# saurabh260918/Graph-Attention-Network-GATv2-

Hardware: AMD Instinct MI355X
Metric: edges/sec (fwd+bwd, 2-layer 8-head GATv2) (higher is better)
Workload: dtype f32; 1 GPU; products-shape synthetic power-law graph, 2450000 nodes / 61900000 edges / 100 feat / 47 classes, 2-layer GATv2 heads [8, 8] outdims [8, 8], fp32; launch=eager, parallelism=single GPU, generator=device (csrc/gat_synth.hip), bit-for-bit synth.py

## Files before the change

### graph-attention-network-gatv2-_amd/csrc/gat_abi.hip

```cpp
#include "gat_internal.h"

#include <algorithm>
#include <cmath>
#include <cstdlib>
#include <cstring>
#include <memory>
#include <mutex>

namespace gat {

static thread_local std::string g_err;
void set_error(const std::string& msg) { g_err = msg; }
int fail(int code, const std::string& msg) {
    g_err = msg;
    return code ? code : GAT_E_INVALID;
}
static std::mutex g_choice_mu;
static std::vector<std::pair<std::string, std::string>> g_choices;
const char* choice_env(const char* name) {
    const char* e = getenv(name);
    if (e) {
        std::lock_guard<std::mutex> lock(g_choice_mu);
        bool seen = false;
        for (auto& kv : g_choices) if (kv.first == name) { kv.second = e; seen = true; }
// ... 935 lines not shown
static bool fused_head(gat_ctx* c) {
    if (c->cfg.keep_taps) return false;
    HeadArgs f{}; HeadBwdArgs b{};
    head_args(c, &f, &b);
    return head_step_supported(b);
}
static int head_step(gat_ctx* c, bool with_gh = true) {
    HeadArgs f{}; HeadBwdArgs b{};
    head_args(c, &f, &b);
    if (!with_gh) b.gh_out = nullptr;
    Scope t(c, GAT_K_HEAD_BWD);
    c->y_valid = false;
    return launch_head_step(f, b, c->stream);
}
static bool fused_last(gat_ctx* c) {
    if (!fused_head(c) || bf16(c) || c->comm || c->n_table != c->n_rows || c->cfg.flat_lrelu_index) return false;
    const Layer& y = c->layers.back();
    if (!edge_fast_path(y.H, y.D, c->n_table) || !y.stash || c->stash == nullptr || c->gH == nullptr) return false;
    if (!edge_last_fused_supported(y.H, y.D, c->cfg.num_classes) || c->dbg != 0) return false;
    static const int env = [] { const char* e = choice_env("GAT_FUSE_LAST"); return e ? (e[0] == '0' ? 0 : 1) : 0; }();
    return env == 1;
}
static int last_layer_fused(gat_ctx* c) {
    const int l = c->cfg.num_layers - 1;
    Layer& y = c->layers[l];
    BwdPlan P;
    GAT_TRY(plan_backward_edges(c, l, &P));
    const EdgeFwdArgs f = plan_forward_edges(c, l);
    const int32_t n_seg = c->work.n_slots;
    float* ga_a = P.a.ga_partial;
    int blocks_a = 0;
    if (n_seg > 0) {
        EdgeFwdArgs fs = f;
        fs.n_items = n_seg;
        {
            Scope t(c, GAT_K_EDGE_FWD);
            GAT_TRY(launch_edge_forward(fs, c->stream));
        }
        {
            Scope t(c, GAT_K_HEAD_BWD);
            GAT_TRY(launch_head_rows(c->slot_info, c->work.n_slots, c->work.n_split, Wo_of(c), y.hout, c->labels_eff ? c->labels_eff : c->labels,
                                     c->gH, c->gh_stride, c->cfg.num_classes, y.D, c->stream));
        }
        EdgeBwdArgs bs = P.a;
        bs.n_items = n_seg;
        bs.ga_partial = ga_a;
        bs.ga_blocks = blocks_a = std::min(1024, edge_backward_blocks(n_seg, y.H, y.D, P.store, false, false, P.stash));
        Scope t(c, GAT_K_EDGE_BWD);
        GAT_TRY(launch_edge_backward(bs, c->stream));
    }
    EdgeLastArgs a{};
    a.f = f; a.f.items = c->items + n_seg; a.f.n_items = c->work.n_items - n_seg;
    float* ga_b = ga_a + (int64_t)blocks_a * y.HD;
    a.b = P.a; a.b.ga_partial = ga_b; a.b.ga_blocks = a.f.n_items > 0 ? std::min(edge_last_fused_blocks(a.f.n_items), 2048 - blocks_a) : 0;
    a.Wo = Wo_of(c); a.labels = c->labels_eff ? c->labels_eff : c->labels; a.gh_out = c->gH; a.C = c->cfg.num_classes;
    {
        Scope t(c, GAT_K_EDGE_FUSED);
        GAT_TRY(launch_edge_last_fused(a, c->stream));
    }
    GAT_TRY(head_step(c, false));
    GAT_TRY(sum_backward_edges(c, l, P));
    Scope t(c, GAT_K_MISC);
    return launch_reduce_partials_add(ga_a, blocks_a + a.b.ga_blocks, y.HD, ga_of(c, l), c->stream);
}
static int overlap_prepare(gat_ctx* c) {
    static const int env = [] { const char* e = choice_env("GAT_OVERLAP"); return e ? (e[0] == '0' ? 0 : 1) : -1; }();
    const int L = c->cfg.num_layers;
    const bool want = env == 1;
    if (!want || L < 2 || c->gPL_bound || c->Xtab) return 0;
    if (!c->gPL_alt) {
        hipStreamCaptureStatus cs = hipStreamCaptureStatusNone;
        (void)hipStreamIsCapturing(c->stream, &cs);
        if (cs != hipStreamCaptureStatusNone) return 0;
        GAT_TRY(dalloc(c, &c->gPL_alt, c->n_table * c->HDmax));
        GAT_TRY(dalloc(c, &c->gPR_alt, c->n_rows * c->HDmax));
        {
            int least = 0, greatest = 0;
            (void)hipDeviceGetStreamPriorityRange(&least, &greatest);
            static const bool prio = [] { const char* e = choice_env("GAT_OVERLAP_PRIO"); return !(e && e[0] == '0'); }();
            if (prio) GAT_HIP(hipStreamCreateWithPriority(&c->side_stream, hipStreamNonBlocking, least));
            else GAT_HIP(hipStreamCreateWithFlags(&c->side_stream, hipStreamNonBlocking));
        }
        for (int l = 0; l < L; ++l) {
            hipEvent_t a, b;
            GAT_HIP(hipEventCreateWithFlags(&a, hipEventDisableTiming));
            GAT_HIP(hipEventCreateWithFlags(&b, hipEventDisableTiming));
            c->ev_fork.push_back(a); c->ev_join.push_back(b);
        }
    }
    return 1;
}
struct OverlapScope {
    gat_ctx* c;
    explicit OverlapScope(gat_ctx* c_, bool on) : c(c_) { c->ov_active = on; }
    ~OverlapScope() { c->ov_active = false; }
};
static int backward_phases(gat_ctx* c, bool head_done = false, bool last_edges_done = false) {
    const int L = c->cfg.num_layers;
    const int ov = last_edges_done ? 0 : overlap_prepare(c);
    if (ov < 0) return ov;
    OverlapScope scope(c, ov == 1);
    std::vector<char> forked((size_t)L, 0);
    if (!head_done) GAT_TRY(gat_head_backward(c));
    for (int l = L - 1; l >= 0; --l) {
        if (ov && l + 2 < L && forked[(size_t)l + 2]) {
            GAT_HIP(hipStreamWaitEvent(c->stream, c->ev_join[(size_t)l + 2], 0));
            forked[(size_t)l + 2] = 0;
// ... 573 lines not shown
```

### graph-attention-network-gatv2-_amd/csrc/gat_edge_kernels.hip

```cpp
#include "gat_internal.h"

#include <map>
#include <mutex>

namespace gat {
namespace {

constexpr float kLog2e = 1.4426950408889634f;
constexpr float kLn2 = 0.6931471805599453f;

__device__ __forceinline__ float lrelu(float v, float s) { return v > 0.f ? v : v * s; }
__device__ __forceinline__ float exp2_fast(float x) { return __builtin_amdgcn_exp2f(x); }

template <int CTRL>
__device__ __forceinline__ float dpp_mov(float v) {
    return __builtin_bit_cast(
        float, __builtin_amdgcn_update_dpp(0, __builtin_bit_cast(int, v), CTRL, 0xF, 0xF, true));
}

template <int D>
__device__ __forceinline__ float group_sum(float t) {
    if constexpr (D >= 2) t += dpp_mov<0xB1>(t);
    if constexpr (D >= 4) t += dpp_mov<0x4E>(t);
    if constexpr (D >= 8) t += dpp_mov<0x141>(t);
// ... 942 lines not shown
            for (int u = 0; u < U; ++u) al[u] = hsum<N>(ac2 * lrelu_n<N>(v[u] + pr, A.slope));
            group_sum_n<DL, U>(al);
#pragma unroll
            for (int u = 0; u < U; ++u) {
                al[u] = exp2_fast(al[u] - m2) * inv;
                ga_[u] = hsum<N>(g * v[u]);
            }
            group_sum_n<DL, U>(ga_);
#pragma unroll
            for (int u = 0; u < U; ++u) {
                const bool valid = b + st * U + u < e;
                const float ge = valid ? al[u] * (ga_[u] - dot) : 0.f;
                const vnf<N> s = v[u] + pr;
                const vnf<N> gs = ge * select_pos<N>(s, ac, acs);
                ga += ge * lrelu_n<N>(s, A.slope);
                gpr += gs;
                if constexpr (MSG) {
                    pend_m[u] = g * al[u] + gs;
                } else {
                    uint32_t bits = 0;
#pragma unroll
                    for (int i = 0; i < N; ++i) bits |= (s[i] > 0.f ? 1u : 0u) << i;
                    const uint32_t w = __builtin_bit_cast(uint32_t, (cp & 1) ? ge : al[u]);
                    pend_w[u] = ((w + (1u << (N - 1))) & ~((1u << N) - 1u)) | bits;
                }
            }
        }
        if constexpr (MSG) {
            if constexpr (DBG != 1) {
#pragma unroll
                for (int u = 0; u < U; ++u) store_row_n<HD, N, BF>(A.msg, (int)pend_s[u], cp, pend_m[u]);
            }
        } else if constexpr (DBG != 1 && DBG != 3) {
#pragma unroll
            for (int u = 0; u < U; ++u) stream_store(&A.stash[(uint64_t)pend_s[u] * LPE + cp], pend_w[u]);
        }
        if (row >= 0) {
            float* dst = slot < 0 ? A.gPR + rowc * HD + c : A.part_acc + (int64_t)slot * HD + c;
            stream_store(reinterpret_cast<vnf<N>*>(dst), gpr);
        }
    }
#pragma unroll
    for (int off = LPE; off < 64; off <<= 1) ga += shfl_xor_n<N>(ga, off);
    if (gidx == 0) {
#pragma unroll
        for (int i = 0; i < N; ++i) red[wave][c + i] = ga[i];
    }
    __syncthreads();
    if (threadIdx.x < HD)
        A.ga_partial[(int64_t)blockIdx.x * HD + threadIdx.x] =
            (red[0][threadIdx.x] + red[1][threadIdx.x]) + (red[2][threadIdx.x] + red[3][threadIdx.x]);
}

template <int HD, int D, int N>
__global__ __launch_bounds__(256) __attribute__((amdgpu_waves_per_eu(4, 8))) void edge_last_fused_kernel(EdgeLastArgs A) {
    constexpr int LPE = HD / N, G = 64 / LPE, DL = D / N, H = HD / D;
    constexpr int U = 4, JC = 4;
    static_assert(LPE == 16 && DL == 2 && D == 8 && N == 4, "16 lanes per row, two lanes per head, D = 8");
    __shared__ float red[4][HD];
    __shared__ float s_wo[64 * D];
    const EdgeFwdArgs& F = A.f;
    const EdgeBwdArgs& B = A.b;
    const int C = A.C;
    for (int i = threadIdx.x; i < C * D; i += blockDim.x) s_wo[i] = A.Wo[i];
    __syncthreads();
    const int lane = threadIdx.x & 63;
    const int wave = __builtin_amdgcn_readfirstlane(threadIdx.x >> 6);
    const int cp = lane % LPE, gidx = lane / LPE;
    const int c = N * cp;
    const vnf<N> ac = *reinterpret_cast<const vnf<N>*>(F.a + c);
    const vnf<N> acs = ac * F.slope;
    const vnf<N> ac2 = ac * kLog2e;
    const int64_t nquads = (F.n_items + G - 1) / G;
    const int64_t nwaves = (int64_t)gridDim.x * 4;
    vnf<N> ga = vzero<N>();

    for (int64_t q = (int64_t)blockIdx.x * 4 + wave; q < nquads; q += nwaves) {
        const int64_t it = q * G + gidx;
        int row = -1, b = 0, e = 0;
        if (it < F.n_items) { const int4 item = F.items[it]; row = item.x; b = item.y; e = item.z; }
        const int64_t rowc = row < 0 ? 0 : row;
        const int nst = wave_max_over_groups<HD, N>((e - b + U - 1) / U);
        const vnf<N> pr = *reinterpret_cast<const vnf<N>*>(F.PR + rowc * HD + c);
        float m = -1e9f * kLog2e, Z = 0.f;
        vnf<N> acc = vzero<N>();
        {
            auto load_src = [&](int st) {
                int j = b + st * U + (cp & (U - 1));
                j = j < e ? j : e - 1;
                return F.col_idx[j > 0 ? j : 0];
            };
            int srcv = load_src(0);
            for (int st = 0; st < nst; ++st) {
                const int srcn = load_src(st + 1);
                vnf<N> v[U];
#pragma unroll
                for (int u = 0; u < U; ++u) v[u] = gather_row_n<HD, N, false>(F.PL, __shfl(srcv, gidx * LPE + u), cp);
                float t[U];
#pragma unroll
                for (int u = 0; u < U; ++u) t[u] = hsum<N>(ac2 * lrelu_n<N>(v[u] + pr, F.slope));
                group_sum_n<DL, U>(t);
                float cm = -INFINITY;
#pragma unroll
                for (int u = 0; u < U; ++u) {
                    t[u] = (b + st * U + u < e) ? t[u] : -INFINITY;
                    cm = fmaxf(cm, t[u]);
                }
                const float mn = fmaxf(m, cm);
                const float scale = exp2_fast(m - mn);
                Z *= scale;
                acc = acc * scale;
#pragma unroll
                for (int u = 0; u < U; ++u) {
                    const float p = exp2_fast(t[u] - mn);
                    Z += p;
                    acc += p * v[u];
                }
                m = mn;
                srcv = srcn;
            }
        }
        const float inv = __builtin_amdgcn_rcpf(Z + 1e-8f);
        const vnf<N> hp = acc * inv;
        if (row >= 0) {
            stream_store(reinterpret_cast<vnf<N>*>(F.hpre + rowc * HD + c), hp);
            if ((c % D) == 0) { F.mstat[rowc * H + c / D] = m; F.zstat[rowc * H + c / D] = Z; }
        }
        vnf<N> hm = lrelu_n<N>(hp, F.slope);
#pragma unroll
        for (int off = DL; off < LPE; off <<= 1) hm += shfl_xor_n<N>(hm, off);
        hm = hm / (float)H;
        if (row >= 0 && cp < DL) *reinterpret_cast<vnf<N>*>(F.hout + rowc * D + c) = hm;
        const vnf<N> ho_other = shfl_xor_n<N>(hm, 1);
        float ho[D];
#pragma unroll
        for (int k = 0; k < N; ++k) { ho[k] = (cp & 1) ? ho_other[k] : hm[k]; ho[N + k] = (cp & 1) ? hm[k] : ho_other[k]; }
        const int lab = A.labels[rowc];
        float z[JC], mv = -INFINITY;
#pragma unroll
        for (int j = 0; j < JC; ++j) {
            const int cls = cp + LPE * j;
            z[j] = -INFINITY;
            if (cls < C) {
                float t = 0.f;
#pragma unroll
                for (int d = 0; d < D; ++d) t += s_wo[cls * D + d] * ho[d];
                z[j] = t;
                mv = fmaxf(mv, t);
            }
        }
#pragma unroll
        for (int off = 1; off < LPE; off <<= 1) mv = fmaxf(mv, __shfl_xor(mv, off));
        float ev[JC], sum = 0.f;
#pragma unroll
        for (int j = 0; j < JC; ++j) { ev[j] = (cp + LPE * j < C) ? exp2_fast((z[j] - mv) * kLog2e) : 0.f; sum += ev[j]; }
        sum = group_sum<LPE>(sum);
        const float rden = 1.0f / (sum + 1e-8f);
        float gh[D];
#pragma unroll
        for (int d = 0; d < D; ++d) gh[d] = 0.f;
#pragma unroll
        for (int j = 0; j < JC; ++j) {
            const int cls = cp + LPE * j;
            if (cls < C) {
                const float dz = lab >= 0 ? ev[j] * rden - (cls == lab ? 1.0f : 0.0f) : 0.0f;
#pragma unroll
                for (int d = 0; d < D; ++d) gh[d] += s_wo[cls * D + d] * dz;
            }
        }
        group_sum_n<LPE, D>(gh);
        vnf<N> ghl;
#pragma unroll
        for (int k = 0; k < N; ++k) ghl[k] = (cp & 1) ? gh[N + k] : gh[k];
        if (row >= 0 && cp < DL) *reinterpret_cast<vnf<N>*>(A.gh_out + rowc * B.gh_stride + c) = ghl;
        vnf<N> dsel;
#pragma unroll
        for (int i = 0; i < N; ++i) dsel[i] = hp[i] > 0.f ? 1.0f : F.slope;
        const vnf<N> g = ghl * dsel * (1.0f / (float)H);
        if (row >= 0) {
            if (B.hbits != nullptr) {
                uint32_t nib = 0;
#pragma unroll
                for (int i = 0; i < N; ++i) nib |= (hp[i] > 0.f ? 1u : 0u) << i;
                B.hbits[rowc * B.hb_stride + cp] = (uint8_t)nib;
            } else {
                stream_store(reinterpret_cast<vnf<N>*>(B.gfull + rowc * HD + c), g);
            }
        }
        const float dot = group_sum<DL>(hsum<N>(g * hp));
        const float m2 = m;
        auto load_idx = [&](int st, int& srcv, int& posv) {
            int j = b + st * U + (cp & (U - 1));
            j = j < e ? j : e - 1;
            j = j > 0 ? j : 0;
            srcv = B.col_idx[j];
            posv = B.pos[j];
        };
        auto spread = [&](int st, int srcv, int posv, int (&src)[U], uint32_t (&sl)[U]) {
#pragma unroll
            for (int u = 0; u < U; ++u) {
                src[u] = __shfl(srcv, gidx * LPE + u);
                const uint32_t p = (uint32_t)__shfl(posv, gidx * LPE + u);
                sl[u] = (b + st * U + u < e) ? p : B.stash_spare;
            }
        };
        int srcv, posv, srcn, posn;
        load_idx(0, srcv, posv);
        load_idx(1, srcn, posn);
        vnf<N> gpr = vzero<N>();
        int src[U];
        uint32_t sl[U], pend_s[U], pend_w[U];
        spread(0, srcv, posv, src, sl);
#pragma unroll
        for (int u = 0; u < U; ++u) { pend_w[u] = 0u; pend_s[u] = B.stash_spare; }
        for (int st = 0; st < nst; ++st) {
            vnf<N> v[U];
#pragma unroll
            for (int u = 0; u < U; ++u) v[u] = gather_row_n<HD, N, false>(B.PL, src[u], cp);
#pragma unroll
            for (int u = 0; u < U; ++u) stream_store(&B.stash[(uint64_t)pend_s[u] * LPE + cp], pend_w[u]);
#pragma unroll
            for (int u = 0; u < U; ++u) pend_s[u] = sl[u];
            spread(st + 1, srcn, posn, src, sl);
            load_idx(st + 2, srcn, posn);
            float al[U], ga_[U];
#pragma unroll
            for (int u = 0; u < U; ++u) al[u] = hsum<N>(ac2 * lrelu_n<N>(v[u] + pr, F.slope));
            group_sum_n<DL, U>(al);
#pragma unroll
            for (int u = 0; u < U; ++u) {
                al[u] = exp2_fast(al[u] - m2) * inv;
                ga_[u] = hsum<N>(g * v[u]);
            }
            group_sum_n<DL, U>(ga_);
#pragma unroll
            for (int u = 0; u < U; ++u) {
                const bool valid = b + st * U + u < e;
                const float ge = valid ? al[u] * (ga_[u] - dot) : 0.f;
                const vnf<N> s = v[u] + pr;
                const vnf<N> gs = ge * select_pos<N>(s, ac, acs);
                ga += ge * lrelu_n<N>(s, F.slope);
                gpr += gs;
                uint32_t bits = 0;
#pragma unroll
                for (int i = 0; i < N; ++i) bits |= (s[i] > 0.f ? 1u : 0u) << i;
                const uint32_t w = __builtin_bit_cast(uint32_t, (cp & 1) ? ge : al[u]);
                pend_w[u] = ((w + (1u << (N - 1))) & ~((1u << N) - 1u)) | bits;
            }
        }
#pragma unroll
        for (int u = 0; u < U; ++u) stream_store(&B.stash[(uint64_t)pend_s[u] * LPE + cp], pend_w[u]);
        if (row >= 0) stream_store(reinterpret_cast<vnf<N>*>(B.gPR + rowc * HD + c), gpr);
    }
#pragma unroll
    for (int off = LPE; off < 64; off <<= 1) ga += shfl_xor_n<N>(ga, off);
    if (gidx == 0) {
#pragma unroll
        for (int i = 0; i < N; ++i) red[wave][c + i] = ga[i];
    }
    __syncthreads();
    if (threadIdx.x < HD)
        B.ga_partial[(int64_t)blockIdx.x * HD + threadIdx.x] =
            (red[0][threadIdx.x] + red[1][threadIdx.x]) + (red[2][threadIdx.x] + red[3][threadIdx.x]);
}

__global__ __launch_bounds__(256) void head_rows_kernel(const int4* __restrict__ slot_info, int32_t n_slots, int32_t n_split,
                                                       const float* __restrict__ Wo, const float* __restrict__ HL,
                                                       const int32_t* __restrict__ labels, float* __restrict__ gh_out,
                                                       int32_t gh_stride, int32_t C, int32_t DLAST) {
    const int k = blockIdx.x * blockDim.x + threadIdx.x;
    if (k >= n_split) return;
    const int64_t row = slot_info[slot_info[n_slots + k].x].x;
    const float* x = HL + row * DLAST;
    const int lab = labels[row];
    float mv = -INFINITY;
    for (int c = 0; c < C; ++c) {
        float t = 0.f;
        for (int d = 0; d < DLAST; ++d) t += Wo[c * DLAST + d] * x[d];
        mv = fmaxf(mv, t);
    }
    float sum = 0.f;
    for (int c = 0; c < C; ++c) {
        float t = 0.f;
        for (int d = 0; d < DLAST; ++d) t += Wo[c * DLAST + d] * x[d];
        sum += exp2_fast((t - mv) * kLog2e);
    }
    const double rden = 1.0 / ((double)sum + 1e-8);
    float acc[16];
    for (int d = 0; d < DLAST; ++d) acc[d] = 0.f;
    for (int c = 0; c < C; ++c) {
        float t = 0.f;
        for (int d = 0; d < DLAST; ++d) t += Wo[c * DLAST + d] * x[d];
        const float y = (float)((double)exp2_fast((t - mv) * kLog2e) * rden);
        const float dz = lab >= 0 ? y - (c == lab ? 1.0f : 0.0f) : 0.0f;
        for (int d = 0; d < DLAST; ++d) acc[d] += Wo[c * DLAST + d] * dz;
    }
    for (int d = 0; d < DLAST; ++d) gh_out[row * gh_stride + d] = acc[d];
}

#ifdef GAT_EXPERIMENTS
template <int NCW, int R>
struct RecRing {
    uint32_t rec[NCW][R][16 * 16];
    uint32_t slot[NCW][R][16];
    int head[NCW], tail[NCW], done[NCW];
// ... 576 lines not shown
    const int dummy = 0;
    auto probe = [&]() -> int {
        GAT_DISPATCH_HD_D(stash_words_t, dummy, nullptr)
        return 0;
    };
    return probe();
}

int edge_backward_blocks(int64_t n_items, int32_t H, int32_t D_, bool store, bool taps, bool bf16, bool stash) {
    int64_t want = (n_items + 3) / 4;
    if (want < 1) want = 1;
    const int HD = H * D_, D = D_;
    const BwdSel sel{store, taps, bf16, stash};
    auto cap = [&]() -> int {
        GAT_DISPATCH_HD_D(bwd_resident, sel, nullptr)
        return 2048;
    };
    int c = cap();
#ifdef GAT_EXPERIMENTS
    static const int dbg = [] { const char* e = getenv("GAT_DBG"); return e ? atoi(e) : 0; }();
    if (dbg == 4 && HD == 64 && D == 8 && stash && !bf16 && !taps) c = c / 2;
#endif
    return (int)(want < c ? want : c);
}

static int fast_probe(const int&, hipStream_t) { return 1; }
template <int HD, int D>
int fast_probe_t(const int& x, hipStream_t s) { return fast_probe(x, s); }

bool edge_fast_path(int32_t H, int32_t D_, int64_t n_table) {
    const int HD = H * D_, D = D_;
    if (n_table * HD * (int64_t)sizeof(float) >= ((int64_t)1 << 32)) return false;
    const int dummy = 0;
    auto probe = [&]() -> int {
        GAT_DISPATCH_HD_D(fast_probe_t, dummy, nullptr)
        return 0;
    };
    return probe() == 1;
}

int launch_edge_backward(const EdgeBwdArgs& a, hipStream_t s) {
    const int HD = a.H * a.D, D = a.D;
    if (a.ga_blocks < 1) return fail(GAT_E_INVALID, "edge_backward: ga_blocks must come from edge_backward_blocks()");
    if (edge_fast_path(a.H, a.D, a.n_table)) { GAT_DISPATCH_HD_D(run_bwd, a, s) }
    if (a.pos != nullptr) return fail(GAT_E_INVALID, "edge_backward: the generic path has no store mode");
    const size_t lds = (size_t)(3 * a.H + 2 * HD) * sizeof(float);
    if (lds > 64 * 1024) return fail(GAT_E_UNSUPPORTED, "edge_backward: H*D too large for the generic path");
    hipLaunchKernelGGL(edge_bwd_generic, dim3((unsigned)a.ga_blocks), dim3(64), lds, s, a);
    GAT_HIP(hipGetLastError());
    return 0;
}

bool edge_last_fused_supported(int32_t H, int32_t D, int32_t C) { return H * D == 64 && D == 8 && C >= 1 && C <= 64; }
int edge_last_fused_blocks(int64_t n_items) {
    const int64_t want = std::max<int64_t>(1, ((n_items + 3) / 4 + 3) / 4);
    const int cap = resident_blocks((const void*)edge_last_fused_kernel<64, 8, 4>);
    return (int)std::min<int64_t>(want, cap);
}
int launch_edge_last_fused(const EdgeLastArgs& a, hipStream_t s) {
    if (!edge_last_fused_supported(a.f.H, a.f.D, a.C)) return fail(GAT_E_UNSUPPORTED, "edge_last_fused: shape outside the kernel");
    if (a.f.n_items <= 0) return 0;
    if (a.f.items == nullptr || a.b.pos == nullptr || a.b.stash == nullptr || a.gh_out == nullptr || a.b.ga_blocks < 1 ||
        (a.b.hbits == nullptr && a.b.gfull == nullptr))
        return fail(GAT_E_INVALID, "edge_last_fused: missing buffers");
    hipLaunchKernelGGL((edge_last_fused_kernel<64, 8, 4>), dim3((unsigned)a.b.ga_blocks), dim3(256), 0, s, a);
    GAT_HIP(hipGetLastError());
    return 0;
}
int launch_head_rows(const int4* slot_info, int32_t n_slots, int32_t n_split, const float* Wo, const float* HL, const int32_t* labels,
                     float* gh_out, int32_t gh_stride, int32_t C, int32_t DLAST, hipStream_t s) {
    if (n_split <= 0) return 0;
    if (DLAST > 16) return fail(GAT_E_UNSUPPORTED, "head_rows: D_last > 16");
    hipLaunchKernelGGL(head_rows_kernel, dim3((unsigned)((n_split + 255) / 256)), dim3(256), 0, s, slot_info, n_slots, n_split, Wo, HL,
                       labels, gh_out, gh_stride, C, DLAST);
    GAT_HIP(hipGetLastError());
    return 0;
}

int launch_csr_to_coo(const int32_t* row_ptr, const int32_t* col_idx, int32_t* src, int32_t* dst,
                      int64_t n_rows, int64_t n_edges, int64_t dst_offset, hipStream_t s) {
    if (n_edges <= 0) return 0;
    int64_t blocks = (n_edges + 255) / 256;
    if (blocks > 65536) blocks = 65536;
    hipLaunchKernelGGL(csr_to_coo_kernel, dim3((unsigned)blocks), dim3(256), 0, s, row_ptr, col_idx, src,
                       dst, n_rows, n_edges, (int32_t)dst_offset);
    GAT_HIP(hipGetLastError());
    return 0;
}

static int launch_transpose(const float* src, float* dst, int64_t A_, int64_t B_, hipStream_t s) {
    const int64_t total = A_ * B_;
    if (total <= 0) return 0;
    int64_t blocks = (total + 255) / 256;
    if (blocks > 65536) blocks = 65536;
    hipLaunchKernelGGL(transpose_kernel, dim3((unsigned)blocks), dim3(256), 0, s, src, dst, A_, B_);
    GAT_HIP(hipGetLastError());
    return 0;
}
int launch_transpose_eh_to_he(const float* src_eh, float* dst_he, int64_t E, int32_t H, hipStream_t s) {
    return launch_transpose(src_eh, dst_he, E, H, s);
}
int launch_transpose_he_to_eh(const float* src_he, float* dst_eh, int64_t E, int32_t H, hipStream_t s) {
    return launch_transpose(src_he, dst_eh, H, E, s);
}
int launch_transpose_nh_to_hn(const float* src_nh, float* dst_hn, int64_t N, int32_t H, hipStream_t s) {
    return launch_transpose(src_nh, dst_hn, N, H, s);
}

}
```

### graph-attention-network-gatv2-_amd/csrc/gat_gemm_kernels.hip

```cpp
#include "gat_internal.h"

#include <cstdlib>
#include <map>
#include <mutex>
#include <utility>

namespace gat {
namespace {

typedef float v16f __attribute__((ext_vector_type(16)));

struct ASrcRows {
    const float* X; int32_t ld;
    __device__ __forceinline__ float4 load4(int64_t i, int k) const {
        return *reinterpret_cast<const float4*>(X + i * ld + k);
    }
    __device__ __forceinline__ float load1(int64_t i, int k) const { return X[i * ld + k]; }
};
struct ASrcGcat {
    const float* gPL; const float* gPR; int32_t HD;
    __device__ __forceinline__ float4 load4(int64_t i, int k) const {
        return k < HD ? *reinterpret_cast<const float4*>(gPL + i * HD + k)
                      : *reinterpret_cast<const float4*>(gPR + i * HD + (k - HD));
    }
// ... 24 lines not shown
    __device__ __forceinline__ void apply(int64_t i, int j, float v, float) const { (*this)(i, j, v); }
    __device__ __forceinline__ void operator()(int64_t i, int j, float v) const {
        j += j0;
        if (j < HD) {
            if constexpr (BF) {
                const uint32_t u = __builtin_bit_cast(uint32_t, v);
                reinterpret_cast<uint16_t*>(PL)[i * HD + j] = (uint16_t)((u + 0x7FFFu + ((u >> 16) & 1u)) >> 16);
            } else {
                PL[i * HD + j] = v;
            }
        } else {
            PR[i * HD + (j - HD)] = v;
        }
    }
};
struct EpiGradX {
    static constexpr bool kTwoPhase = true;
    float* out; const float* hpre_prev; int32_t ld; float slope;
    __device__ __forceinline__ float pre(int64_t i, int j) const { return hpre_prev[i * ld + j]; }
    __device__ __forceinline__ void apply(int64_t i, int j, float v, float hv) const {
        out[i * ld + j] = v * (hv > 0.f ? 1.0f : slope);
    }
    __device__ __forceinline__ void operator()(int64_t i, int j, float v) const { apply(i, j, v, pre(i, j)); }
};

struct EpiStore {
    static constexpr bool kTwoPhase = false;
    float* out; int32_t ld;
    __device__ __forceinline__ float pre(int64_t, int) const { return 0.f; }
    __device__ __forceinline__ void apply(int64_t i, int j, float v, float) const { out[i * ld + j] = v; }
    __device__ __forceinline__ void operator()(int64_t i, int j, float v) const { out[i * ld + j] = v; }
};

constexpr int kKC = 128;

}

int64_t resident_blocks(const void* fn, size_t dyn_lds, int threads) {
    static std::mutex mu;
    static std::map<std::pair<const void*, size_t>, int64_t> cache;
    std::lock_guard<std::mutex> lock(mu);
    const auto key = std::make_pair(fn, dyn_lds);
    auto it = cache.find(key);
    if (it != cache.end()) return it->second;
    int per_cu = 0, dev = 0, cus = 256;
    if (hipOccupancyMaxActiveBlocksPerMultiprocessor(&per_cu, fn, threads, dyn_lds) != hipSuccess || per_cu < 1) per_cu = 1;
    if (per_cu > 8) per_cu = 8;
    (void)hipGetDevice(&dev);
    (void)hipDeviceGetAttribute(&cus, hipDeviceAttributeMultiprocessorCount, dev);
    (void)hipGetLastError();
    return cache[key] = (int64_t)per_cu * (cus > 0 ? cus : 256);
}

static void allow_big_lds(const void* fn) {
    static std::mutex mu;
    static std::map<std::pair<const void*, int>, bool> done;
    int dev = 0;
    (void)hipGetDevice(&dev);
    std::lock_guard<std::mutex> lock(mu);
    bool& d = done[std::make_pair(fn, dev)];
    if (!d) { (void)hipFuncSetAttribute(fn, hipFuncAttributeMaxDynamicSharedMemorySize, 160 * 1024); (void)hipGetLastError(); d = true; }
}

namespace {

template <int NT, bool VEC4, class AS, class BS, class EP>
__global__ __launch_bounds__(256) void rowgemm_kernel(AS as, BS bs, EP ep, int64_t M, int32_t N, int32_t K,
                                                      int32_t kc_lds) {
    constexpr int NW = NT * 32;
    extern __shared__ float Bsh[];
    const int lane = threadIdx.x & 63, wave = threadIdx.x >> 6;
    const int li = lane & 31, half = lane >> 5;
    const int n0 = blockIdx.y * NW;
    const int64_t ntiles = (M + 127) / 128;
    bool b_loaded = false;
    for (int64_t tile = blockIdx.x; tile < ntiles; tile += gridDim.x) {
        const int64_t row = tile * 128 + wave * 32 + li;
        const bool rvalid = row < M;
        v16f acc[NT];
#pragma unroll
        for (int nt = 0; nt < NT; ++nt)
#pragma unroll
            for (int r = 0; r < 16; ++r) acc[nt][r] = 0.f;
        for (int k0 = 0; k0 < K; k0 += kKC) {
            const int kc = (K - k0 < kKC) ? (K - k0) : kKC;
            const int kc8 = (kc + 7) & ~7;
            if (K > kKC || !b_loaded) {
                __syncthreads();
                if constexpr (BS::kAlongK) {
                    for (int idx = threadIdx.x; idx < kc8 * NW; idx += 256) {
                        const int kk = idx % kc8, j = idx / kc8;
                        Bsh[kk * NW + j] = (kk < kc && n0 + j < N) ? bs.at(k0 + kk, n0 + j) : 0.f;
                    }
                } else {
                    for (int idx = threadIdx.x; idx < kc8 * NW; idx += 256) {
                        const int kk = idx / NW, j = idx % NW;
                        Bsh[kk * NW + j] = (kk < kc && n0 + j < N) ? bs.at(k0 + kk, n0 + j) : 0.f;
                    }
                }
                b_loaded = true;
                __syncthreads();
            }
            float4 af[kKC / 8];
#pragma unroll
            for (int st = 0; st < kKC / 8; ++st) {
                const int kk = st * 8 + 4 * half;
                af[st] = make_float4(0.f, 0.f, 0.f, 0.f);
// ... 930 lines not shown
```

### graph-attention-network-gatv2-_amd/csrc/gat_internal.h

```cpp
#pragma once
#include <hip/hip_runtime.h>
#include <cstdint>
#include <cstdio>
#include <string>
#include <vector>

#include "gatv2_abi.h"

namespace gat {

constexpr int kWave = 64;

void set_error(const std::string& msg);
int fail(int code, const std::string& msg);
const char* choice_env(const char* name);

#define GAT_HIP(expr)                                                                     \
    do {                                                                                  \
        hipError_t e__ = (expr);                                                          \
        if (e__ != hipSuccess)                                                            \
            return ::gat::fail((int)e__, std::string(#expr) + ": " + hipGetErrorString(e__)); \
    } while (0)

#define GAT_TRY(expr)                 \
// ... 38 lines not shown
    int32_t n_split = 0;
};
void build_worklist(const int32_t* row_ptr, int64_t n_rows, WorkList& w);
int launch_edge_forward(const EdgeFwdArgs& a, hipStream_t s);

struct EdgeBwdArgs {
    const int32_t* row_ptr;
    const int32_t* col_idx;
    const float* PL;
    const float* PR;
    const float* a;
    const float* alpha;
    const float* mstat;
    const float* zstat;
    const float* hpre;
    const float* g;
    int32_t g_raw;
    const float* gh;
    float* gPL;
    const int32_t* pos;
    float* msg;
    uint32_t* stash;
    uint32_t stash_spare;
    float* gfull;
    int32_t gh_stride;
    int32_t hb_stride;
    uint8_t* hbits;
    float* gPR;
    float* ge;
    float* galpha;
    float* ga_partial;
    int32_t ga_blocks;
    int64_t n_rows;
    int64_t n_table;
    int32_t bf16;
    int32_t H, D;
    float slope;
    const int4* items;
    int64_t n_items;
    const int4* slot_info;
    int32_t n_slots;
    int32_t n_split;
    float* part_acc;
    int32_t dbg;
};
int launch_edge_backward(const EdgeBwdArgs& a, hipStream_t s);
struct EdgeLastArgs {
    EdgeFwdArgs f;
    EdgeBwdArgs b;
    const float* Wo;
    const int32_t* labels;
    float* gh_out;
    int32_t C;
};
bool edge_last_fused_supported(int32_t H, int32_t D, int32_t C);
int edge_last_fused_blocks(int64_t n_items);
int launch_edge_last_fused(const EdgeLastArgs& a, hipStream_t s);
int launch_head_rows(const int4* slot_info, int32_t n_slots, int32_t n_split, const float* Wo, const float* HL, const int32_t* labels,
                     float* gh_out, int32_t gh_stride, int32_t C, int32_t DLAST, hipStream_t s);
int edge_stash_words(int32_t H, int32_t D);
int edge_backward_blocks(int64_t n_items, int32_t H, int32_t D, bool store, bool taps, bool bf16, bool stash = false);
bool edge_fast_path(int32_t H, int32_t D, int64_t n_table);

int build_csc(const int32_t* col_idx, int64_t n_edges, int64_t n_table, int32_t* pos, int32_t* src_ptr,
              int32_t* csrc, hipStream_t s);
struct HeavyList {
    std::vector<int32_t> chunks;
    std::vector<int32_t> heavy;
    int32_t threshold = 0;
    std::vector<int32_t> items;
    int32_t run = 0; int64_t n_runs = 0;
    std::vector<int32_t> open;
    std::vector<int32_t> empty;
};
int build_heavy_list(const int32_t* d_src_ptr, int64_t n_table, int64_t n_edges, HeavyList* out, hipStream_t s, int32_t run = 0);
struct SlotRuns {
    const int32_t* csrc = nullptr;
    int32_t run = 0;
    int64_t n_runs = 0;
    const int4* open = nullptr; int32_t n_open = 0;
    const int32_t* empty = nullptr; int64_t n_empty = 0;
    float* part = nullptr;
};
int launch_gpl_sum(const int32_t* src_ptr, const float* msg, float* gPL, int64_t n_table, int64_t n_slots,
                   int32_t HD, bool msg_bf16, const int4* chunks, int32_t n_chunks, const int4* heavy,
                   int32_t n_heavy, float* part, hipStream_t s, const SlotRuns* runs = nullptr);
constexpr int64_t kPullPad = 32;
int build_csc_dst(const int32_t* row_ptr, const int32_t* pos, int32_t* cdst, int64_t n_rows, int64_t n_edges, hipStream_t s);
int launch_gpl_pull(const int32_t* src_ptr, const uint32_t* stash, const int32_t* cdst, const float* gfull, bool g_bf16,
                    const float* gh, const uint8_t* hbits, int32_t gh_stride, int32_t hb_stride, const float* a,
                    float slope, float* gPL, int64_t n_table, int64_t n_slots, int32_t H, int32_t D, const int4* chunks,
                    int32_t n_chunks, const int4* heavy, int32_t n_heavy, float* part, const int4* items, int64_t n_items, const SlotRuns* runs,
                    int64_t slot_capacity , hipStream_t s);

int launch_csr_to_coo(const int32_t* row_ptr, const int32_t* col_idx, int32_t* src, int32_t* dst,
                      int64_t n_rows, int64_t n_edges, int64_t table_row0, hipStream_t s);

struct Comm {
    int world = 1, rank = 0;
    virtual ~Comm();
    virtual int all_gather(float* table, int64_t slice, hipStream_t s) = 0;
    virtual int all_gather_part(float* table, int64_t slice, int64_t off, int64_t cnt, hipStream_t s) = 0;
    virtual int reduce_scatter(float* table, int64_t slice, hipStream_t s) = 0;
    virtual int reduce_scatter_bf16(float* table, int64_t slice, hipStream_t s) = 0;
    virtual int all_reduce(float* buf, int64_t n, hipStream_t s) = 0;
    virtual int exchange_rows(const float* sendbuf, const int64_t* cnt_send, float* recvbuf, const int64_t* cnt_recv, int64_t rf, hipStream_t s) = 0;
};
struct HaloPlan {
    int world = 0, rank = 0;
    int64_t max_rows = 0;
    std::vector<int64_t> need_cnt, send_cnt;
    int64_t n_need = 0, n_send = 0, buf_rows = 0;
    int32_t* need_rows = nullptr;
    int32_t* send_rows = nullptr;
    int32_t *arr_ptr = nullptr, *arr_split = nullptr, *arr_pos = nullptr;
    float *sendbuf = nullptr, *recvbuf = nullptr;
    double referenced_fraction = 1.0;
};
int halo_build(Comm* comm, const int32_t* d_col_idx, int64_t n_edges, int64_t n_table, int32_t hd_max, HaloPlan* out, hipStream_t s);
int halo_forward(Comm* comm, const HaloPlan& h, float* table, int64_t rf, hipStream_t s);
int halo_backward(Comm* comm, const HaloPlan& h, float* gPL, int64_t rf, hipStream_t s);
void halo_free(HaloPlan* h);
int comm_unique_id(void* id_out);
int comm_create_rccl(int world, int rank, const void* id_bytes, Comm** out);
int comm_create_host(int world, int rank, const char* shm_name, int64_t bytes_per_rank, Comm** out);

int launch_pack_result(const float* loss, const int32_t* correct, float* dst3, hipStream_t s);
struct ReduceJob { const float* slabs; float* out; int64_t width; int32_t nslabs, HD, F, c_base, block0; };
struct ReduceBatch {
    ReduceJob jobs[8]; int32_t n, blocks;
    const float* loss; const int32_t* correct; float* dst3; float* dst3_host;
    const double* fin_loss; const int32_t* fin_corr; int32_t fin_n; float* fin_loss_out; int32_t* fin_corr_out;
};
void reduce_batch_begin();
void reduce_batch_abort();
void reduce_batch_pack(const float* loss, const int32_t* correct, float* dst3, float* dst3_host);
bool reduce_batch_finalize(const double* loss_partial, const int32_t* correct_partial, int32_t nblocks, float* loss_out, int32_t* correct_out);
int reduce_batch_flush(hipStream_t s);
int launch_reduce_partials_add(const float* partial, int32_t nblocks, int64_t width, float* out,
                               hipStream_t s);

int launch_reduce_gradw(const float* slabs, int32_t ksplit, int32_t HD, int32_t F, int32_t c_base, int32_t M,
                        float* gradW, hipStream_t s);

int64_t resident_blocks(const void* fn, size_t dyn_lds, int threads = 256);

int launch_transpose_eh_to_he(const float* src_eh, float* dst_he, int64_t E, int32_t H, hipStream_t s);
int launch_transpose_he_to_eh(const float* src_he, float* dst_eh, int64_t E, int32_t H, hipStream_t s);
int launch_transpose_nh_to_hn(const float* src_nh, float* dst_hn, int64_t N, int32_t H, hipStream_t s);

enum : int32_t { kPartBoth = 0, kPartLeft = 1, kPartRight = 2 };
int64_t project_scratch_floats(int64_t n_rows, int32_t F, int32_t HD, int32_t part);
int launch_project(const float* X, const float* W, float* PL_rows, float* PR, int64_t n_rows,
                   int32_t F, int32_t HD, int32_t part, bool pl_bf16, float* scratch, int64_t scratch_floats, hipStream_t s, int32_t ldx = 0);
int64_t grad_w_scratch_floats(int64_t n_rows, int32_t F, int32_t HD);
int launch_grad_w(const float* gPL_rows, const float* gPR, const float* X, float* gradW,
                  float* scratch, int64_t n_rows, int32_t F, int32_t HD, int32_t part, hipStream_t s, int32_t ldx = 0);
int launch_grad_x(const float* gPL_rows, const float* gPR, const float* W, const float* hpre_prev,
                  float* gprev, int64_t n_rows, int32_t F, int32_t HD, float slope, hipStream_t s);

struct HeadArgs {
    const float* Wo;
    const float* HL;
    const int32_t* labels;
    float* y;
    double* loss_partial;
    int32_t* correct_partial;
    float* loss_out;
    int32_t* correct_out;
    int64_t n_rows;
    int32_t C, DL;
};
int head_blocks(int64_t n_rows);
int launch_head_forward(const HeadArgs& a, hipStream_t s);

struct HeadBwdArgs {
    const float* Wo;
    const float* HL;
    const float* y;
    const int32_t* labels;
    const float* hpre;
    float* g;
    float* gh_out;
    int32_t gh_stride;
    float* gradWo;
    float* partial;
    int64_t n_rows;
    int32_t C, DL, H;
    float slope;
    int32_t flat_index;
};
int head_bwd_blocks(int64_t n_rows, int32_t C, int32_t DL);
int launch_head_backward(const HeadBwdArgs& a, hipStream_t s);
bool head_step_supported(const HeadBwdArgs& b);
int launch_head_step(const HeadArgs& f, const HeadBwdArgs& b, hipStream_t s);

int launch_apply_mask(const int32_t* labels, const uint8_t* mask, int32_t* eff, int64_t n, hipStream_t s);
int launch_eval_mask(const float* y, const int32_t* labels, const uint8_t* mask, int64_t n, int32_t C, double* part_loss,
// ... 9 lines not shown
```

Baseline: 2.946 billion edges/s.

## Cache first gathered neighbor rows in LDS ring for fused last-layer backward

The fused last-layer edge kernel now stores the first ring_k gathered PL rows per item (default 8 edges) in a dynamic LDS ring during the forward softmax pass. The backward pass reads those rows back from LDS instead of gathering them from global memory again, and skips the matching col_idx loads. The change also switches address arithmetic to 32-bit offsets and replaces shuffles in the head/softmax section with ds_swizzle and bitmask selects. The added dynamic LDS (up to 32KB per block at default) may reduce resident blocks per CU and so occupancy.

Result: no change. 2.943 billion edges/s (median of 2 runs) (-0.1%).

```diff
diff --git a/graph-attention-network-gatv2-_amd/csrc/gat_abi.hip b/graph-attention-network-gatv2-_amd/csrc/gat_abi.hip
--- a/graph-attention-network-gatv2-_amd/csrc/gat_abi.hip
+++ b/graph-attention-network-gatv2-_amd/csrc/gat_abi.hip
@@ -1011,7 +1011,8 @@
     EdgeLastArgs a{};
     a.f = f; a.f.items = c->items + n_seg; a.f.n_items = c->work.n_items - n_seg;
     float* ga_b = ga_a + (int64_t)blocks_a * y.HD;
-    a.b = P.a; a.b.ga_partial = ga_b; a.b.ga_blocks = a.f.n_items > 0 ? std::min(edge_last_fused_blocks(a.f.n_items), 2048 - blocks_a) : 0;
+    a.ring_k = edge_last_ring_edges();
+    a.b = P.a; a.b.ga_partial = ga_b; a.b.ga_blocks = a.f.n_items > 0 ? std::min(edge_last_fused_blocks(a.f.n_items, a.ring_k), 2048 - blocks_a) : 0;
     a.Wo = Wo_of(c); a.labels = c->labels_eff ? c->labels_eff : c->labels; a.gh_out = c->gH; a.C = c->cfg.num_classes;
     {
         Scope t(c, GAT_K_EDGE_FUSED);
diff --git a/graph-attention-network-gatv2-_amd/csrc/gat_edge_kernels.hip b/graph-attention-network-gatv2-_amd/csrc/gat_edge_kernels.hip
--- a/graph-attention-network-gatv2-_amd/csrc/gat_edge_kernels.hip
+++ b/graph-attention-network-gatv2-_amd/csrc/gat_edge_kernels.hip
@@ -1018,6 +1018,26 @@
             (red[0][threadIdx.x] + red[1][threadIdx.x]) + (red[2][threadIdx.x] + red[3][threadIdx.x]);
 }
 
+template <class T>
+__device__ __forceinline__ T* at32(T* base, uint32_t elem) {
+    return reinterpret_cast<T*>(reinterpret_cast<typename std::conditional<std::is_const<T>::value, const char, char>::type*>(base) +
+                                elem * (uint32_t)sizeof(T));
+}
+template <int OFF>
+__device__ __forceinline__ float xor_swz(float v) {
+    static_assert(OFF > 0 && OFF < 32, "ds_swizzle bit mode works inside 32 lanes");
+    return __builtin_bit_cast(float, __builtin_amdgcn_ds_swizzle(__builtin_bit_cast(int, v), (OFF << 10) | 0x1F));
+}
+template <int OFF, int N>
+__device__ __forceinline__ vnf<N> xor_swz_n(vnf<N> v) {
+    vnf<N> r;
+#pragma unroll
+    for (int i = 0; i < N; ++i) r[i] = xor_swz<OFF>(v[i]);
+    return r;
+}
+__device__ __forceinline__ float pick(uint32_t odd_mask, float a, float b) {
+    return __builtin_bit_cast(float, (__builtin_bit_cast(uint32_t, a) & odd_mask) | (__builtin_bit_cast(uint32_t, b) & ~odd_mask));
+}
 template <int HD, int D, int N>
 __global__ __launch_bounds__(256) __attribute__((amdgpu_waves_per_eu(4, 8))) void edge_last_fused_kernel(EdgeLastArgs A) {
     constexpr int LPE = HD / N, G = 64 / LPE, DL = D / N, H = HD / D;
@@ -1025,15 +1045,19 @@
     static_assert(LPE == 16 && DL == 2 && D == 8 && N == 4, "16 lanes per row, two lanes per head, D = 8");
     __shared__ float red[4][HD];
     __shared__ float s_wo[64 * D];
+    extern __shared__ float4 last_ring[];
     const EdgeFwdArgs& F = A.f;
     const EdgeBwdArgs& B = A.b;
     const int C = A.C;
-    for (int i = threadIdx.x; i < C * D; i += blockDim.x) s_wo[i] = A.Wo[i];
+    for (int i = threadIdx.x; i < 64 * D; i += blockDim.x) s_wo[i] = i < C * D ? A.Wo[i] : 0.f;
     __syncthreads();
     const int lane = threadIdx.x & 63;
     const int wave = __builtin_amdgcn_readfirstlane(threadIdx.x >> 6);
     const int cp = lane % LPE, gidx = lane / LPE;
     const int c = N * cp;
+    const uint32_t odd = (cp & 1) ? 0xFFFFFFFFu : 0u;
+    const int KS = A.ring_k / U;
+    vnf<N>* const ring = reinterpret_cast<vnf<N>*>(last_ring) + wave * A.ring_k * 64 + lane;
     const vnf<N> ac = *reinterpret_cast<const vnf<N>*>(F.a + c);
     const vnf<N> acs = ac * F.slope;
     const vnf<N> ac2 = ac * kLog2e;
@@ -1045,9 +1069,9 @@
         const int64_t it = q * G + gidx;
         int row = -1, b = 0, e = 0;
         if (it < F.n_items) { const int4 item = F.items[it]; row = item.x; b = item.y; e = item.z; }
-        const int64_t rowc = row < 0 ? 0 : row;
+        const uint32_t rowc = row < 0 ? 0u : (uint32_t)row;
         const int nst = wave_max_over_groups<HD, N>((e - b + U - 1) / U);
-        const vnf<N> pr = *reinterpret_cast<const vnf<N>*>(F.PR + rowc * HD + c);
+        const vnf<N> pr = *at32(reinterpret_cast<const vnf<N>*>(F.PR), rowc * (HD / N) + cp);
         float m = -1e9f * kLog2e, Z = 0.f;
         vnf<N> acc = vzero<N>();
         {
@@ -1062,6 +1086,10 @@
                 vnf<N> v[U];
 #pragma unroll
                 for (int u = 0; u < U; ++u) v[u] = gather_row_n<HD, N, false>(F.PL, __shfl(srcv, gidx * LPE + u), cp);
+                if (st < KS) {
+#pragma unroll
+                    for (int u = 0; u < U; ++u) ring[(st * U + u) * 64] = v[u];
+                }
                 float t[U];
 #pragma unroll
                 for (int u = 0; u < U; ++u) t[u] = hsum<N>(ac2 * lrelu_n<N>(v[u] + pr, F.slope));
@@ -1089,56 +1117,56 @@
         const float inv = __builtin_amdgcn_rcpf(Z + 1e-8f);
         const vnf<N> hp = acc * inv;
         if (row >= 0) {
-            stream_store(reinterpret_cast<vnf<N>*>(F.hpre + rowc * HD + c), hp);
-            if ((c % D) == 0) { F.mstat[rowc * H + c / D] = m; F.zstat[rowc * H + c / D] = Z; }
-        }
-        vnf<N> hm = lrelu_n<N>(hp, F.slope);
-#pragma unroll
-        for (int off = DL; off < LPE; off <<= 1) hm += shfl_xor_n<N>(hm, off);
-        hm = hm / (float)H;
-        if (row >= 0 && cp < DL) *reinterpret_cast<vnf<N>*>(F.hout + rowc * D + c) = hm;
-        const vnf<N> ho_other = shfl_xor_n<N>(hm, 1);
-        float ho[D];
-#pragma unroll
-        for (int k = 0; k < N; ++k) { ho[k] = (cp & 1) ? ho_other[k] : hm[k]; ho[N + k] = (cp & 1) ? hm[k] : ho_other[k]; }
-        const int lab = A.labels[rowc];
-        float z[JC], mv = -INFINITY;
-#pragma unroll
-        for (int j = 0; j < JC; ++j) {
-            const int cls = cp + LPE * j;
-            z[j] = -INFINITY;
-            if (cls < C) {
+            stream_store(at32(reinterpret_cast<vnf<N>*>(F.hpre), rowc * (HD / N) + cp), hp);
+            if ((c % D) == 0) { *at32(F.mstat, rowc * H + c / D) = m; *at32(F.zstat, rowc * H + c / D) = Z; }
+        }
+        vnf<N> ghl;
+        {
+            static_assert(DL == 2 && LPE == 16, "the head's lane exchanges below");
+            vnf<N> hm = lrelu_n<N>(hp, F.slope);
+            hm += xor_swz_n<2, N>(hm);
+            hm += xor_swz_n<4, N>(hm);
+            hm += xor_swz_n<8, N>(hm);
+            hm = hm / (float)H;
+            if (row >= 0 && cp < DL) *at32(reinterpret_cast<vnf<N>*>(F.hout), rowc * (D / N) + cp) = hm;
+            const vnf<N> ho_other = xor_swz_n<1, N>(hm);
+            float ho[D];
+#pragma unroll
+            for (int k = 0; k < N; ++k) { ho[k] = pick(odd, ho_other[k], hm[k]); ho[N + k] = pick(odd, hm[k], ho_other[k]); }
+            const int lab = *at32(A.labels, rowc);
+            const float* wo = s_wo + cp * D;
+            float z[JC], mv = -INFINITY;
+#pragma unroll
+            for (int j = 0; j < JC; ++j) {
                 float t = 0.f;
 #pragma unroll
-                for (int d = 0; d < D; ++d) t += s_wo[cls * D + d] * ho[d];
-                z[j] = t;
-                mv = fmaxf(mv, t);
-            }
-        }
-#pragma unroll
-        for (int off = 1; off < LPE; off <<= 1) mv = fmaxf(mv, __shfl_xor(mv, off));
-        float ev[JC], sum = 0.f;
-#pragma unroll
-        for (int j = 0; j < JC; ++j) { ev[j] = (cp + LPE * j < C) ? exp2_fast((z[j] - mv) * kLog2e) : 0.f; sum += ev[j]; }
-        sum = group_sum<LPE>(sum);
-        const float rden = 1.0f / (sum + 1e-8f);
-        float gh[D];
-#pragma unroll
-        for (int d = 0; d < D; ++d) gh[d] = 0.f;
-#pragma unroll
-        for (int j = 0; j < JC; ++j) {
-            const int cls = cp + LPE * j;
-            if (cls < C) {
-                const float dz = lab >= 0 ? ev[j] * rden - (cls == lab ? 1.0f : 0.0f) : 0.0f;
-#pragma unroll
-                for (int d = 0; d < D; ++d) gh[d] += s_wo[cls * D + d] * dz;
-            }
-        }
-        group_sum_n<LPE, D>(gh);
-        vnf<N> ghl;
-#pragma unroll
-        for (int k = 0; k < N; ++k) ghl[k] = (cp & 1) ? gh[N + k] : gh[k];
-        if (row >= 0 && cp < DL) *reinterpret_cast<vnf<N>*>(A.gh_out + rowc * B.gh_stride + c) = ghl;
+                for (int d = 0; d < D; ++d) t += wo[j * LPE * D + d] * ho[d];
+                z[j] = cp < C - LPE * j ? t : -INFINITY;
+                mv = fmaxf(mv, z[j]);
+            }
+            mv = fmaxf(mv, xor_swz<1>(mv));
+            mv = fmaxf(mv, xor_swz<2>(mv));
+            mv = fmaxf(mv, xor_swz<4>(mv));
+            mv = fmaxf(mv, xor_swz<8>(mv));
+            float sum = 0.f;
+#pragma unroll
+            for (int j = 0; j < JC; ++j) { z[j] = cp < C - LPE * j ? exp2_fast((z[j] - mv) * kLog2e) : 0.f; sum += z[j]; }
+            sum = group_sum<LPE>(sum);
+            const float rden = 1.0f / (sum + 1e-8f);
+            float gh[D];
+#pragma unroll
+            for (int d = 0; d < D; ++d) gh[d] = 0.f;
+#pragma unroll
+            for (int j = 0; j < JC; ++j) {
+                const float dz = (lab >= 0 && cp < C - LPE * j) ? z[j] * rden - (cp == lab - LPE * j ? 1.0f : 0.0f) : 0.0f;
+#pragma unroll
+                for (int d = 0; d < D; ++d) gh[d] += wo[j * LPE * D + d] * dz;
+            }
+            group_sum_n<LPE, D>(gh);
+#pragma unroll
+            for (int k = 0; k < N; ++k) ghl[k] = pick(odd, gh[N + k], gh[k]);
+        }
+        if (row >= 0 && cp < DL) *reinterpret_cast<vnf<N>*>(at32(A.gh_out, rowc * (uint32_t)B.gh_stride + c)) = ghl;
         vnf<N> dsel;
 #pragma unroll
         for (int i = 0; i < N; ++i) dsel[i] = hp[i] > 0.f ? 1.0f : F.slope;
@@ -1148,9 +1176,9 @@
                 uint32_t nib = 0;
 #pragma unroll
                 for (int i = 0; i < N; ++i) nib |= (hp[i] > 0.f ? 1u : 0u) << i;
-                B.hbits[rowc * B.hb_stride + cp] = (uint8_t)nib;
+                *at32(B.hbits, rowc * (uint32_t)B.hb_stride + cp) = (uint8_t)nib;
             } else {
-                stream_store(reinterpret_cast<vnf<N>*>(B.gfull + rowc * HD + c), g);
+                stream_store(at32(reinterpret_cast<vnf<N>*>(B.gfull), rowc * (HD / N) + cp), g);
             }
         }
         const float dot = group_sum<DL>(hsum<N>(g * hp));
@@ -1159,7 +1187,7 @@
             int j = b + st * U + (cp & (U - 1));
             j = j < e ? j : e - 1;
             j = j > 0 ? j : 0;
-            srcv = B.col_idx[j];
+            srcv = st >= KS ? B.col_idx[j] : 0;
             posv = B.pos[j];
         };
         auto spread = [&](int st, int srcv, int posv, int (&src)[U], uint32_t (&sl)[U]) {
@@ -1179,10 +1207,15 @@
         spread(0, srcv, posv, src, sl);
 #pragma unroll
         for (int u = 0; u < U; ++u) { pend_w[u] = 0u; pend_s[u] = B.stash_spare; }
-        for (int st = 0; st < nst; ++st) {
+        auto bstep = [&](auto from_ring, int st) {
             vnf<N> v[U];
-#pragma unroll
-            for (int u = 0; u < U; ++u) v[u] = gather_row_n<HD, N, false>(B.PL, src[u], cp);
+            if constexpr (decltype(from_ring)::value) {
+#pragma unroll
+                for (int u = 0; u < U; ++u) v[u] = ring[(st * U + u) * 64];
+            } else {
+#pragma unroll
+                for (int u = 0; u < U; ++u) v[u] = gather_row_n<HD, N, false>(B.PL, src[u], cp);
+            }
 #pragma unroll
             for (int u = 0; u < U; ++u) stream_store(&B.stash[(uint64_t)pend_s[u] * LPE + cp], pend_w[u]);
 #pragma unroll
@@ -1213,10 +1246,14 @@
                 const uint32_t w = __builtin_bit_cast(uint32_t, (cp & 1) ? ge : al[u]);
                 pend_w[u] = ((w + (1u << (N - 1))) & ~((1u << N) - 1u)) | bits;
             }
-        }
+        };
+        const int nr = nst < KS ? nst : KS;
+        int st = 0;
+        for (; st < nr; ++st) bstep(std::true_type{}, st);
+        for (; st < nst; ++st) bstep(std::false_type{}, st);
 #pragma unroll
         for (int u = 0; u < U; ++u) stream_store(&B.stash[(uint64_t)pend_s[u] * LPE + cp], pend_w[u]);
-        if (row >= 0) stream_store(reinterpret_cast<vnf<N>*>(B.gPR + rowc * HD + c), gpr);
+        if (row >= 0) stream_store(at32(reinterpret_cast<vnf<N>*>(B.gPR), rowc * (HD / N) + cp), gpr);
     }
 #pragma unroll
     for (int off = LPE; off < 64; off <<= 1) ga += shfl_xor_n<N>(ga, off);
@@ -1899,18 +1936,33 @@
 }
 
 bool edge_last_fused_supported(int32_t H, int32_t D, int32_t C) { return H * D == 64 && D == 8 && C >= 1 && C <= 64; }
-int edge_last_fused_blocks(int64_t n_items) {
+int edge_last_ring_edges() {
+    static const int v = [] {
+        const char* e = choice_env("GAT_LAST_RING");
+        if (!e) return 8;
+        const int k = atoi(e);
+        return (k >= 0 && k <= 32 && k % 4 == 0) ? k : 8;
+    }();
+    return v;
+}
+static size_t last_ring_lds(int ring_k) { return (size_t)ring_k * 4 * 64 * sizeof(float4); }
+int edge_last_fused_blocks(int64_t n_items, int ring_k) {
     const int64_t want = std::max<int64_t>(1, ((n_items + 3) / 4 + 3) / 4);
-    const int cap = resident_blocks((const void*)edge_last_fused_kernel<64, 8, 4>);
+    const void* fn = (const void*)edge_last_fused_kernel<64, 8, 4>;
+    if (ring_k > 0) allow_big_lds(fn);
+    const int64_t cap = resident_blocks(fn, last_ring_lds(ring_k), 256);
     return (int)std::min<int64_t>(want, cap);
 }
 int launch_edge_last_fused(const EdgeLastArgs& a, hipStream_t s) {
     if (!edge_last_fused_supported(a.f.H, a.f.D, a.C)) return fail(GAT_E_UNSUPPORTED, "edge_last_fused: shape outside the kernel");
+    if (a.ring_k < 0 || a.ring_k > 32 || a.ring_k % 4 != 0) return fail(GAT_E_INVALID, "edge_last_fused: ring_k must be 0, 4, ... 32");
     if (a.f.n_items <= 0) return 0;
     if (a.f.items == nullptr || a.b.pos == nullptr || a.b.stash == nullptr || a.gh_out == nullptr || a.b.ga_blocks < 1 ||
         (a.b.hbits == nullptr && a.b.gfull == nullptr))
         return fail(GAT_E_INVALID, "edge_last_fused: missing buffers");
-    hipLaunchKernelGGL((edge_last_fused_kernel<64, 8, 4>), dim3((unsigned)a.b.ga_blocks), dim3(256), 0, s, a);
+    const void* fn = (const void*)edge_last_fused_kernel<64, 8, 4>;
+    if (a.ring_k > 0) allow_big_lds(fn);
+    hipLaunchKernelGGL((edge_last_fused_kernel<64, 8, 4>), dim3((unsigned)a.b.ga_blocks), dim3(256), last_ring_lds(a.ring_k), s, a);
     GAT_HIP(hipGetLastError());
     return 0;
 }
diff --git a/graph-attention-network-gatv2-_amd/csrc/gat_gemm_kernels.hip b/graph-attention-network-gatv2-_amd/csrc/gat_gemm_kernels.hip
--- a/graph-attention-network-gatv2-_amd/csrc/gat_gemm_kernels.hip
+++ b/graph-attention-network-gatv2-_amd/csrc/gat_gemm_kernels.hip
@@ -100,7 +100,7 @@
     return cache[key] = (int64_t)per_cu * (cus > 0 ? cus : 256);
 }
 
-static void allow_big_lds(const void* fn) {
+void allow_big_lds(const void* fn) {
     static std::mutex mu;
     static std::map<std::pair<const void*, int>, bool> done;
     int dev = 0;
diff --git a/graph-attention-network-gatv2-_amd/csrc/gat_internal.h b/graph-attention-network-gatv2-_amd/csrc/gat_internal.h
--- a/graph-attention-network-gatv2-_amd/csrc/gat_internal.h
+++ b/graph-attention-network-gatv2-_amd/csrc/gat_internal.h
@@ -114,9 +114,11 @@
     const int32_t* labels;
     float* gh_out;
     int32_t C;
+    int32_t ring_k;
 };
 bool edge_last_fused_supported(int32_t H, int32_t D, int32_t C);
-int edge_last_fused_blocks(int64_t n_items);
+int edge_last_ring_edges();
+int edge_last_fused_blocks(int64_t n_items, int ring_k);
 int launch_edge_last_fused(const EdgeLastArgs& a, hipStream_t s);
 int launch_head_rows(const int4* slot_info, int32_t n_slots, int32_t n_split, const float* Wo, const float* HL, const int32_t* labels,
                      float* gh_out, int32_t gh_stride, int32_t C, int32_t DLAST, hipStream_t s);
@@ -206,6 +208,7 @@
                         float* gradW, hipStream_t s);
 
 int64_t resident_blocks(const void* fn, size_t dyn_lds, int threads = 256);
+void allow_big_lds(const void* fn);
 
 int launch_transpose_eh_to_he(const float* src_eh, float* dst_he, int64_t E, int32_t H, hipStream_t s);
 int launch_transpose_he_to_eh(const float* src_he, float* dst_eh, int64_t E, int32_t H, hipStream_t s);
```
